# ariasanovsky/azdopt

Measured on AMD Instinct MI355X. Metric: node_expansions_per_s, higher is better.
Workload: dtype f32

## Files before the change

azdopt_amd/_lib.py:

```python
import ctypes as C
import os
import subprocess

_HERE = os.path.dirname(os.path.abspath(__file__))
LIB_PATH = os.environ.get("AZD_LIB", os.path.join(_HERE, "libazdopt_amd.so"))
_LIB = None

CTR = dict(EXPANSIONS=0, TERMINALS=1, TRANSPOSITIONS=2, VISITED_STEPS=3, SELECT_CALLS=4, SUM_DEG=5,
           SUM_ACTIONS=6, CASCADE_NODES=7, NEW_PREDS=8, ROOT_EXHAUSTED=9, MAX_FRONTIER=10, MAX_DEPTH=11,
           CURIOSITY_PAIRS=12, EVAL_LAYER_CLOCKS=13, TICKS_ADD_ACTIONS=14, FAILED=15, TICKS_TOTAL=16, TICKS_SELECT=17, TICKS_LOOKUP=18, TICKS_NEWNODE=19,
           TICKS_CASCADE=20, TICKS_MAX_CALL=21, TICKS_LAMBDA=22, TICKS_MATCHING=23, TICKS_WAIT=24, EVAL_BATCHES=25, EVAL_ROWS=26, EVAL_TILES=27, TICKS_TILES=28, TICKS_BATCH=29, TICKS_TILE_SETUP=30, TICKS_TILE_KLOOP=31)
CTR_COUNT = 32

ACT_NONE, ACT_RELU, ACT_SIGMOID = 0, 1, 2
ENGINE_NO_PERSISTENT_STEP = 1
ENGINE_ASYNC_STEP = 2
ENGINE_BARRIER_STEP = 4
ENGINE_POOL_STEP = 8
ENGINE_DENSE_AH = 32
ENGINE_RAMSEY_U64 = 16
ENGINE_EXT_POOL_STEP = 64
SPACE_C21 = 1
SPACE_RAMSEY = 2
SPACE_DENSE = 3
# ... 107 lines not shown
    sig("azd_evaluator_destroy", C.c_int, vp)
    sig("azd_evaluator_write_predictions", C.c_int, vp, C.c_int, vp, vp)
    sig("azd_evaluator_update_model", C.c_int, vp, C.c_int, vp, vp, vp, f32p)
    sig("azd_evaluator_write_predictions_dev", C.c_int, vp, C.c_int, vp, vp, vp)
    sig("azd_evaluator_update_model_dev", C.c_int, vp, C.c_int, vp, vp, vp, f32p, vp)
    sig("azd_evaluator_set_weight_storage", C.c_int, vp, C.c_int)
    sig("azd_evaluator_num_params", C.c_int64, vp)
    sig("azd_evaluator_get_params", C.c_int, vp, vp)
    sig("azd_evaluator_set_params", C.c_int, vp, vp)
    sig("azd_evaluator_calls", C.c_uint64, vp)
    sig("azd_engine_create", C.c_int, C.POINTER(vp), C.POINTER(EngineConfig), vp)
    sig("azd_engine_destroy", C.c_int, vp)
    sig("azd_engine_par_new", C.c_int, vp, vp, vp)
    sig("azd_engine_par_roll_out_episodes", C.c_int, vp, vp, C.c_int, C.c_uint32, C.c_int, i32p)
    sig("azd_engine_run_ahead", C.c_int, vp, vp, C.c_int, C.c_uint32, C.c_int, i32p)
    sig("azd_engine_par_update_model", C.c_int, vp, C.c_uint32, f32p)
    sig("azd_engine_par_update_model_sharded", C.c_int, vp, C.c_uint32, vp, f32p)
    sig("azd_engine_par_reset_trees", C.c_int, vp, vp, vp)
    sig("azd_engine_argmin_data", C.c_int, vp, C.POINTER(Argmin))
    sig("azd_engine_agent_counters", C.c_int, vp, vp)
    sig("azd_engine_agent_counters_per_agent", C.c_int, vp)
    sig("azd_engine_pool_agent_finish", C.c_int, vp, vp)
    sig("azd_engine_pool_groups", C.c_int, vp, vp, vp, vp)
    sig("azd_engine_ramsey_argmin_data", C.c_int, vp, C.POINTER(RamseyArgmin))
    sig("azd_engine_ramsey_wide_argmin_data", C.c_int, vp, C.POINTER(RamseyWideArgmin))
    sig("azd_engine_ramsey_argmin_any", C.c_int, vp, vp, C.c_int, vp, C.c_int, vp, f32p, i32p, C.POINTER(C.c_uint32))
    sig("azd_engine_ramsey_agent_counts", C.c_int, vp, C.c_int, vp, vp)
    sig("azd_ramsey_state_dim", C.c_int, C.c_int, C.c_int)
    sig("azd_ramsey_action_dim", C.c_int, C.c_int, C.c_int)
    sig("azd_ramsey_key_words", C.c_int, C.c_int, C.c_int)
    sig("azd_ramsey_generate_roots", C.c_int, C.c_uint64, C.c_uint64, C.c_uint64, C.c_int, C.c_int, C.c_int, C.c_int,
        C.c_int, vp, vp)
    sig("azd_ramsey_generate_roots_weighted", C.c_int, C.c_uint64, C.c_uint64, C.c_uint64, C.c_int, C.c_int, C.c_int, C.c_int,
        C.c_int, vp, vp, vp)
    sig("azd_engine_set_root_policy", C.c_int, vp, C.POINTER(RootPolicy))
    sig("azd_engine_get_root_policy", C.c_int, vp, C.POINTER(RootPolicy))
    sig("azd_root_policy_check", C.c_int, C.c_int, C.c_int, C.POINTER(RootPolicy))
    sig("azd_engine_root_policy_report", C.c_int, vp, vp, vp, vp)
    sig("azd_dense_state_dim", C.c_int, C.c_int)
    sig("azd_dense_action_dim", C.c_int, C.c_int)
    sig("azd_dense_key_words", C.c_int, C.c_int)
    sig("azd_dense_generate_roots", C.c_int, C.c_uint64, C.c_uint64, C.c_uint64, C.c_int, C.c_int, C.c_int, C.c_int, C.c_double, vp, vp)
    sig("azd_engine_dense_argmin_data", C.c_int, vp, C.POINTER(DenseArgmin))
    sig("azd_c21_modify_roots", C.c_int, vp, C.c_uint64, C.c_uint64, C.c_int, C.c_int, vp, vp)
    sig("azd_c21_modify_roots_dev", C.c_int, vp, C.c_uint64, C.c_uint64, C.c_int, C.c_int, vp, vp)
    sig("azd_engine_par_reset_trees_c21", C.c_int, vp, C.c_uint64, C.c_uint64, C.c_int, C.c_int)
# ... 47 lines not shown
```

azdopt_amd/csrc/async_step.inc:

```

struct AsyncCtl {
    uint32_t req[PERSIST_WAVES];
    uint32_t rows[PERSIST_WAVES];
    uint32_t nrows;
    uint32_t lock;
    uint32_t active;
    uint32_t gen;
    uint32_t tile_next[8];
    uint32_t tile_done[8];
    uint32_t finished;
    uint32_t prog[PERSIST_WAVES];
    unsigned long long t_open;
};

#define LDS_LOAD(p) __hip_atomic_load((p), __ATOMIC_RELAXED, __HIP_MEMORY_SCOPE_WORKGROUP)
#define LDS_STORE(p, v) __hip_atomic_store((p), (v), __ATOMIC_RELAXED, __HIP_MEMORY_SCOPE_WORKGROUP)
#define WG_RELEASE() __builtin_amdgcn_fence(__ATOMIC_RELEASE, "workgroup")
#define WG_ACQUIRE() __builtin_amdgcn_fence(__ATOMIC_ACQUIRE, "workgroup")

struct EvalPtrs {
    const void *__restrict__ wpk;
    const float *__restrict__ params;
    const float *state_vecs;
    float *h_theta;
};

__device__ __forceinline__ float *row_lds(const uint32_t owner_wave, const uint32_t dyn_stride) {
    return reinterpret_cast<float *>(lds_base(owner_wave * dyn_stride) + 16u * owner_wave);
}

typedef short bf16x4 __attribute__((ext_vector_type(4)));

struct AsyncRows {
    AsyncCtl &ctl;
    uint32_t dyn_stride;
    int t0;
    __device__ __forceinline__ int count() const { return (int)LDS_LOAD(&ctl.nrows); }
    __device__ __forceinline__ float *row(const int r) const { return row_lds(LDS_LOAD(&ctl.rows[r]), dyn_stride); }
    __device__ __forceinline__ int agent(const int r) const { return t0 + (int)LDS_LOAD(&ctl.rows[r]); }
    __device__ __forceinline__ float *out(const int) const { return nullptr; }
};

#ifndef AZD_MLP_PF
#define AZD_MLP_PF 8
#endif
constexpr int MLP_PF = AZD_MLP_PF;
template <class Rows, bool LAST_TO_LDS = false>
__device__ void mlp_tile_task(const FusedEval &ev, const Rows &rows, const EvalPtrs &gp, const int l, const int tile,
                              unsigned long long *ph) {
    ph[0] = PH_NOW();
    const int lane = LANE;
    const int L = ev.n_layers;
    const int K = ev.dims[l], N = ev.dims[l + 1];
    const int S4 = (ev.dims[0] + 15) & ~15, H = ev.hid[0];
    const int nrows = rows.count();
    const int n0 = tile * 16;
    const int r = lane & 15;
    const int rr = r < nrows ? r : 0;
    float *const rbase = rows.row(rr);
    const float *arow = rbase + (l == 0 ? 0 : S4 + ((l - 1) & 1) * H);
    const float *ap = arow + 4 * (lane >> 4);
    f32x4 acc = {0.f, 0.f, 0.f, 0.f};
    const int steps = (K + 15) >> 4;
    const size_t frag = (size_t)ev.p_off[l] + ((size_t)tile * steps * 64 + lane) * 4;
    ph[1] = PH_NOW();
    if (ev.bf16) {
        const uint16_t *wq = reinterpret_cast<const uint16_t *>(gp.wpk) + frag;
        const uint16_t *ap16 = reinterpret_cast<const uint16_t *>(rbase) + (l == 0 ? 0 : S4 + ((l - 1) & 1) * H) + 4 * (lane >> 4);
        int s0 = 0;
        for (; s0 + MLP_PF <= steps; s0 += MLP_PF) {
            uint2 bq[MLP_PF], aq[MLP_PF];
#pragma unroll
            for (int j = 0; j < MLP_PF; ++j) bq[j] = *reinterpret_cast<const uint2 *>(wq + 256 * (s0 + j));
#pragma unroll
            for (int j = 0; j < MLP_PF; ++j) aq[j] = *reinterpret_cast<const uint2 *>(ap16 + 16 * (s0 + j));
            __builtin_amdgcn_sched_barrier(0);
#pragma unroll
            for (int j = 0; j < MLP_PF; ++j) {
                bf16x4 a4, b4;
                __builtin_memcpy(&a4, &aq[j], 8);
                __builtin_memcpy(&b4, &bq[j], 8);
                acc = __builtin_amdgcn_mfma_f32_16x16x16bf16_1k(a4, b4, acc, 0, 0, 0);
            }
        }
        if (s0 < steps) {
            uint2 bq[MLP_PF];
#pragma unroll
            for (int j = 0; j < MLP_PF; ++j)
                if (s0 + j < steps) bq[j] = *reinterpret_cast<const uint2 *>(wq + 256 * (s0 + j));
            __builtin_amdgcn_sched_barrier(0);
#pragma unroll
            for (int j = 0; j < MLP_PF; ++j)
                if (s0 + j < steps) {
                    const uint2 bv = bq[j];
                    const uint2 ab = *reinterpret_cast<const uint2 *>(ap16 + 16 * (s0 + j));
                    bf16x4 a4, b4;
                    __builtin_memcpy(&a4, &ab, 8);
                    __builtin_memcpy(&b4, &bv, 8);
                    acc = __builtin_amdgcn_mfma_f32_16x16x16bf16_1k(a4, b4, acc, 0, 0, 0);
                }
        }
    } else {
        const float *wp = reinterpret_cast<const float *>(gp.wpk) + frag;
        int s0 = 0;
        for (; s0 + MLP_PF <= steps; s0 += MLP_PF) {
            float4 bq[MLP_PF];
#pragma unroll
            for (int j = 0; j < MLP_PF; ++j) bq[j] = *reinterpret_cast<const float4 *>(wp + 256 * (s0 + j));
            float4 a0 = *reinterpret_cast<const float4 *>(ap + 16 * s0);
            float4 a1 = *reinterpret_cast<const float4 *>(ap + 16 * (s0 + 1));
            __builtin_amdgcn_sched_barrier(0);
#pragma unroll
            for (int j = 0; j < MLP_PF; ++j) {
                float4 a2 = a1;
                if (j + 2 < MLP_PF) a2 = *reinterpret_cast<const float4 *>(ap + 16 * (s0 + j + 2));
                acc = __builtin_amdgcn_mfma_f32_16x16x4f32(a0.x, bq[j].x, acc, 0, 0, 0);
                acc = __builtin_amdgcn_mfma_f32_16x16x4f32(a0.y, bq[j].y, acc, 0, 0, 0);
                acc = __builtin_amdgcn_mfma_f32_16x16x4f32(a0.z, bq[j].z, acc, 0, 0, 0);
                acc = __builtin_amdgcn_mfma_f32_16x16x4f32(a0.w, bq[j].w, acc, 0, 0, 0);
                __builtin_amdgcn_sched_barrier(0);
                a0 = a1;
                a1 = a2;
            }
        }
        if (s0 < steps) {
            float4 bq[MLP_PF];
#pragma unroll
// ... 304 lines not shown
```

azdopt_amd/csrc/engine.hip:

```cpp
#include <hip/hip_runtime.h>

#include <dlfcn.h>

#include <algorithm>
#include <cstdio>
#include <cstring>
#include <new>
#include <string>
#include <vector>

#include "../../include/azdopt_amd.h"
#include "c21_host.h"
#include "engine_types.h"
#include "evaluator.h"
#include "space_ops.h"

namespace azd {

thread_local std::string g_last_error;

int hip_fail(hipError_t e, const char *what) {
    g_last_error = std::string(what) + ": " + hipGetErrorString(e);
    if (e == hipErrorNoDevice || e == hipErrorInvalidDevice) return AZD_ERR_NO_DEVICE;
    if (e == hipErrorOutOfMemory) return AZD_ERR_OUT_OF_MEMORY;
// ... 200 lines not shown
    unsigned long long *d_ext_t0 = nullptr;
    int ext_depth = 2;
    hipEvent_t ext_done = nullptr, ext_fork = nullptr, ext_ring[EXT_STREAMS][EXT_IN_FLIGHT] = {};
    unsigned long long ext_iterations = 0;
    const struct ExtPoolForm *ext = nullptr;
    uint16_t *ext_s16 = nullptr;
    int ext_s16_pitch = 0;
    int kw_host = 0;
    int ramsey_slots = 0;
    int dense_slots = 0;
    uint64_t *d_stage_slots = nullptr;
    azd_root_policy root_policy{AZD_ROOT_RULE_THRESHOLD, 0, {0.0, 0.0, 0.0, 0.0}};
    azd::RootPolicyArgs root_args{};
    uint32_t *d_root_report = nullptr;
    uint32_t *root_report = nullptr;
    bool root_report_valid = false;
    std::vector<uint64_t> dense_packed;
    std::vector<uint64_t> ramsey_perm_pad;
    bool pool_step = false;
    azd::PoolArgs pool{};
    size_t pool_slot_words = 0;
    int n_cus = 0;
    int pool_eval_wgs = 0, pool_search_wgs = 0;
    int pool_grp_g = 0, pool_grp_groups = 0, pool_grp_w = 0;
    int pool_search_waves = 0;
    double pool_util_eval = 0, pool_util_search = 0;
    struct {
        int n_eval = 0;
        int updates = 0;
    } pool_fb;
    struct Window {
        bool open = false;
        bool drained = false;
        bool lumped = false;
        int n = 0, consumed = 0;
        azd::TolTable tol{};
        uint32_t best_ord = 0;
        unsigned long long best_key = ~0ull;
        unsigned long long side_key = ~0ull;
        unsigned long long base_improved = 0;
        unsigned long long reported = 0;
        azd::FusedEval fe{};
        azd::PoolArgs pool{};
    } win;
    unsigned long long *h_win_log = nullptr;
    uint32_t *h_win_flag = nullptr;
// ... 1069 lines not shown
        e->step_reason = xf.r_no_wg;
        return AZD_OK;
    }
    int n_ext = xf.streams;
    if (const char *env = getenv(xf.env_streams)) n_ext = atoi(env);
    n_ext = n_ext < 1 ? 1 : n_ext > azd_engine::EXT_STREAMS ? azd_engine::EXT_STREAMS : n_ext;
    if (!e->ext_done) AZD_HIP(hipEventCreateWithFlags(&e->ext_done, hipEventDisableTiming));
    if (!e->ext_fork) AZD_HIP(hipEventCreateWithFlags(&e->ext_fork, hipEventDisableTiming));
    for (int x = 0; x < n_ext; ++x) {
        if (!e->ext_stream[x]) AZD_HIP(hipStreamCreateWithFlags(&e->ext_stream[x], hipStreamNonBlocking));
        for (int i = 0; i < azd_engine::EXT_IN_FLIGHT; ++i)
            if (!e->ext_ring[x][i]) AZD_HIP(hipEventCreateWithFlags(&e->ext_ring[x][i], hipEventDisableTiming));
    }
    azd::PoolArgs pool = e->pool;
    pool.n_eval = 0;
    pool.ready_lanes = 0;
    pool.n_express = 0;
    pool.express_waves = 0;
    pool.express_shift = 0;
    pool.early_post = xf.early_post;
    if (const char *env = getenv("AZD_POOL_EARLY_POST")) pool.early_post = atoi(env);
    pool.eval_stride = pool.eval_out_off = 0;
    pool.eval_rows = 0;
    pool.debug_abort_call = 0;
    if (const char *env = getenv("AZD_POOL_DEBUG_ABORT_CALL")) pool.debug_abort_call = (uint32_t)atoi(env);
    if (!hashed) {
        const int st_r = e->ev->ensure_rows(n_ext * a.B);
        if (st_r) return st_r;
    }
    int rounds = 4;
    if (const char *env = getenv(xf.env_rounds)) rounds = atoi(env);
    rounds = rounds < 1 ? 1 : rounds > 16 ? 16 : rounds;
    const uint64_t layout = e->ev->layout_version + (hashed ? 1ull << 63 : 0ull) + ((uint64_t)rounds << 56);
    if (e->ext_graph_n != n_ext || e->ext_graph_layout != layout) {
        for (int x = 0; x < azd_engine::EXT_STREAMS; ++x)
            if (e->ext_graph[x]) {
                (void)hipGraphExecDestroy(e->ext_graph[x]);
                e->ext_graph[x] = nullptr;
            }
        e->ext_graph_n = 0;
        for (int x = 0; x < n_ext; ++x) {
            uint32_t *rows = e->d_ext_rows + (size_t)x * a.B, *home = e->d_ext_home + (size_t)x * a.B, *cnt = e->d_ext_n + x;
            hipGraph_t g = nullptr;
            AZD_HIP(hipStreamBeginCapture(e->ext_stream[x], hipStreamCaptureModeThreadLocal));
            int st_g = AZD_OK;
            for (int r = 0; r < rounds && st_g == AZD_OK; ++r) {
// ... 224 lines not shown
            }
            n_eval = n_eval < 1 ? 1 : n_eval;
            if (pool_feedback_on() && e->pool_fb.n_eval > 0) {
                const int fb = e->pool_fb.n_eval;
                const int want_search = (B + 7) / 8, most = want_search < e->n_cus / 2 ? e->n_cus - want_search : e->n_cus / 2;
                n_eval = fb > cap ? cap : fb;
                n_eval = n_eval > most ? most : n_eval;
                n_eval = n_eval < 1 ? 1 : n_eval;
            }
            if (n_calls <= 64 && fe.kind == 3) {
                const int want_search = (B + 7) / 8, most = want_search < e->n_cus / 2 ? e->n_cus - want_search : e->n_cus / 2;
                n_eval += n_eval / 7;
                n_eval = n_eval > most ? most : n_eval;
                n_eval = n_eval > cap ? cap : n_eval;
            }
            if (const char *env = getenv("AZD_POOL_EVAL_WGS")) n_eval = atoi(env) > 0 ? atoi(env) : n_eval;
        }
        int n_search = e->n_cus - n_eval;
        const int want = (B + 7) / 8;
        n_search = n_search > want ? want : n_search;
        n_search = n_search < 1 ? 1 : n_search;
        if (const char *env = getenv("AZD_POOL_SEARCH_WGS")) n_search = atoi(env) > 0 ? atoi(env) : n_search;
        int capacity = e->ops->pool_max_resident(e->a, dyn_bytes, e->n_cus);
        if (const char *env = getenv("AZD_POOL_MAX_RESIDENT")) capacity = atoi(env);
        if (fe.kind < 3) n_eval = 0;
        if (n_eval + n_search > capacity) {
            if (n_eval > capacity / 2) n_eval = capacity / 2;
            if (fe.kind >= 3 && n_eval < 1) n_eval = 1;
            n_search = capacity - n_eval;
        }
        if (n_search < 1 || capacity < 1) {
            use_pool = false;
            char buf[160];
            snprintf(buf, sizeof(buf), "pool step: the device holds %d of its workgroups at once; it needs an evaluator and a searcher resident together; ", capacity);
            e->step_reason = buf;
        }
        pool.n_eval = n_eval;
        pool.ready_lanes = 0;
        if (const char *env = getenv("AZD_POOL_READY_LANES")) pool.ready_lanes = atoi(env);
        pool.n_express = (fe.kind >= 3 && n_search >= 64) ? 8 : 0;
        pool.express_waves = 8;
        pool.express_shift = 4;
        if (const char *env = getenv("AZD_POOL_EXPRESS_WGS")) pool.n_express = atoi(env);
        if (const char *env = getenv("AZD_POOL_EXPRESS_WAVES")) pool.express_waves = (uint32_t)atoi(env);
        if (const char *env = getenv("AZD_POOL_EXPRESS_SHIFT")) pool.express_shift = (uint32_t)atoi(env);
        if (pool.n_express > n_search / 2) pool.n_express = n_search / 2;
// ... 57 lines not shown
                    e->grp_lds_host = gpl.lds;
                }
                pool.grp_g = gpl.g;
                pool.grp_w = gpl.W;
                pool.grp_groups = n_groups;
                pool.grp_tile = e->d_grp_tile;
                pool.grp_lds = e->d_grp_lds;
                pool.grp_desc = e->d_grp_desc;
                pool.grp_cnt = e->d_grp_cnt;
                pool.grp_x = e->d_grp_x;
                pool.grp_flag = e->d_grp_flag;
                pool.grp_xstride = gpl.xstride;
                n_eval = n_groups * gpl.g;
                pool.n_eval = n_eval;
                if (gpl.lds_bytes > dyn_bytes) dyn_bytes = gpl.lds_bytes;
            }
        }
        pool_blocks = n_eval + n_search;
        e->pool_grp_g = pool.grp_g;
        e->pool_grp_groups = pool.grp_groups;
        e->pool_grp_w = pool.grp_w;
        e->pool_eval_wgs = n_eval;
        e->pool_search_wgs = n_search;
        e->pool_search_waves = (n_search - pool.n_express) * 16 + pool.n_express * (int)pool.express_waves;
    }
    if (e->pool_step && fusable && !use_pool) {
        use_async = !e->barrier_step && e->ops->async_plan(e->a, fe, &dyn_stride, &dyn_bytes, &why_a);
        use_barrier = !use_async && e->ops->persist_plan(e->a, fe, &dyn_stride, &dyn_bytes, &why_b);
        if (!use_async) e->step_reason += why_a;
        if (!use_async && !use_barrier && *why_b) e->step_reason += std::string("; ") + why_b;
    }
    e->step_form = use_pool ? AZD_STEP_POOL : use_async ? AZD_STEP_ASYNC : use_barrier ? AZD_STEP_BARRIER : AZD_STEP_PER_CALL;
    if (e->a.space == azd::SPACE_DENSE)
        e->step_reason = dense_reason.empty() ? "AZD_DENSE_NO_POOL: the dense-graph space's pool step was switched off" : dense_reason;
    if (ext_ramsey) e->step_reason = ext_demoted || e->step_reason.empty() ? ext_reason : ext_reason + "; " + e->step_reason;
    if (ahead) {
        const bool ok = use_pool && fe.kind >= 3 && n_calls >= 1 && n_calls <= e->log_calls && !e->timing;
        if (!ok) return AZD_OK;
        *accepted = 1;
    }
    if (use_pool || use_async || use_barrier) {
        auto send_args = [&](const azd::PoolArgs &pl) -> int {
            azd::PersistArgs &pa = e->pargs_sent;
            azd::PersistArgs now;
            memset(&now, 0, sizeof(now));
            now.a = e->a;
// ... 1028 lines not shown
    return AZD_OK;
}
int azd_engine_timing(azd_engine *e, double *tree_ms, double *evaluator_ms, uint64_t *tree_launches) {
    if (!e) return AZD_ERR_INVALID_ARGUMENT;
    if (tree_ms) *tree_ms = e->rollout_ms;
    if (evaluator_ms) *evaluator_ms = e->evaluator_ms;
    if (tree_launches) *tree_launches = e->rollout_launches;
    return AZD_OK;
}
void *azd_engine_stream(azd_engine *e) { return e ? (void *)e->stream : nullptr; }
int azd_engine_pool_utilisation(azd_engine *e, double *eval_busy, double *search_busy) {
    if (!e) return AZD_ERR_INVALID_ARGUMENT;
    if (eval_busy) *eval_busy = e->pool_util_eval;
    if (search_busy) *search_busy = e->pool_util_search;
    return AZD_OK;
}
int azd_engine_pool_groups(azd_engine *e, int *members, int *groups, int *waves_per_slot) {
    if (!e) return AZD_ERR_INVALID_ARGUMENT;
    if (members) *members = e->pool_grp_g;
    if (groups) *groups = e->pool_grp_groups;
    if (waves_per_slot) *waves_per_slot = e->pool_grp_w;
    return AZD_OK;
}
int azd_engine_pool_agent_finish(azd_engine *e, uint64_t *ticks_out) {
    if (!e || !ticks_out) return AZD_ERR_INVALID_ARGUMENT;
    AZD_ENTER(e);
    if (!e->pool.stamp) {
        azd::g_last_error = "pool_agent_finish: this engine has run no pool step";
        return AZD_ERR_INVALID_ARGUMENT;
    }
    AZD_HIP(hipStreamSynchronize(e->stream));
    AZD_HIP(hipMemcpy(ticks_out, e->pool.stamp, (size_t)e->a.B * 8, hipMemcpyDeviceToHost));
    return AZD_OK;
}
int azd_engine_pool_split(azd_engine *e, int *eval_wgs, int *search_wgs) {
    if (!e) return AZD_ERR_INVALID_ARGUMENT;
    if (eval_wgs) *eval_wgs = e->pool_eval_wgs;
    if (search_wgs) *search_wgs = e->pool_search_wgs;
    return AZD_OK;
}
int azd_debug_probe_xcc(int device, uint32_t *out, int n_blocks) {
    if (!out || n_blocks <= 0) return AZD_ERR_INVALID_ARGUMENT;
    int st = azd::device_ok(device);
    if (st) return st;
    AZD_HIP(hipSetDevice(device));
    uint32_t *d = nullptr;
// ... 271 lines not shown
```

azdopt_amd/csrc/engine_types.h:

```cpp
#pragma once
#include <stddef.h>
#include <stdint.h>

namespace azd {

constexpr uint32_t NONE = 0xFFFFFFFFu;
constexpr int PARENTS_STRIDE = 32;
constexpr int MAX_N = 24;
constexpr int MAX_KW = 6;
constexpr int PATH_SET = 0, PATH_SEQUENCE = 1;
constexpr int SPACE_C21 = 1, SPACE_RAMSEY = 2, SPACE_DENSE = 3;
constexpr int PRED_CHUNKS = 2;
constexpr int MAX_NODE_ACTIONS = 64 * PRED_CHUNKS;
constexpr int RAMSEY_U64_KW = 36;
constexpr int RAMSEY_U64_CH = 8;
constexpr int FRONTIER_CAP = 256;
constexpr int PATH_STACK = 32;
constexpr int MAX_TOL = 32;
constexpr int NUM_COUNTERS = 32;

struct __attribute__((aligned(16))) NodeRec {
    float c_star;
    uint32_t nt_ex;
    float c;
// ... 224 lines not shown
struct PendRec {
    uint32_t pos;
    float c;
    uint32_t n_preds;
    uint32_t call;
};
struct PoolArgs {
    PoolCtl *ctl;
    uint32_t *ready_slots;
    uint32_t *eval_slots;
    int ready_lanes;
    int n_express;
    uint32_t express_waves;
    uint32_t express_shift;
    int early_post;
    uint32_t qcap;
    uint32_t *join;
    PendRec *pend;
    unsigned long long *stamp;
    int n_eval;
    uint32_t eval_stride;
    uint32_t eval_out_off;
    uint32_t eval_rows;
    uint32_t *post_call;
    int grp_g, grp_w, grp_groups;
    const int16_t *grp_tile;
    const uint32_t *grp_lds;
    uint32_t *grp_desc;
    uint32_t *grp_cnt;
    uint32_t *grp_flag;
    float *grp_x;
    uint32_t grp_xstride;
    uint32_t debug_abort_call;
    uint32_t *win_count;
    unsigned long long *win_log;
    uint32_t *win_flag;
};

struct StepLaunch {
    int n_calls;
    unsigned long long *log_key;
    const uint32_t *resume;
    PoolCtl *ctl;
    int hashed;
    int groups = 0;
    int window;
// ... 11 lines not shown
```

azdopt_amd/csrc/pool_step.inc:

```

constexpr unsigned long long POOL_WAIT_TICKS = 400000000ull;
struct PoolWait {
    unsigned long long t0;
    uint32_t polls;
    __device__ __forceinline__ PoolWait() : t0(0), polls(0) {}
    __device__ __forceinline__ bool expired() {
        if ((++polls & 255u) != 0u) return false;
        const unsigned long long now = (unsigned long long)wall_clock64();
        if (t0 == 0) t0 = now;
        return now - t0 > POOL_WAIT_TICKS;
    }
};

__device__ __forceinline__ uint32_t pool_xcc_id() {
    uint32_t v;
    asm volatile("s_getreg_b32 %0, hwreg(HW_REG_XCC_ID)" : "=s"(v));
    return v & 7u;
}

#ifndef AZD_POOL_FILL_WAIT
#define AZD_POOL_FILL_WAIT 2
#endif
#ifndef AZD_POOL_FILL_SLEEP
#define AZD_POOL_FILL_SLEEP 32
// ... 29 lines not shown
#define POOL_FLUSH_PER_AGENT(A, S, T) ((void)0)
#endif
#ifndef AZD_POOL_EXPRESS_SLACK
#define AZD_POOL_EXPRESS_SLACK 2
#endif
#ifndef AZD_POOL_STANDBY
#define AZD_POOL_STANDBY 4
#endif
constexpr int POOL_BATCH_MAX = 32;
struct PoolBatch {
    uint32_t agent[POOL_BATCH_MAX];
    uint32_t home[POOL_BATCH_MAX];
    uint32_t n, first[2], cnt[2], q, leave;
};

struct PoolRows {
    uint32_t stride, out_off;
    const uint32_t *agents;
    int n;
    __device__ __forceinline__ int count() const { return n; }
    __device__ __forceinline__ float *row(const int r) const { return reinterpret_cast<float *>(lds_base((uint32_t)r * stride * 4u)); }
    __device__ __forceinline__ int agent(const int r) const { return (int)agents[r]; }
    __device__ __forceinline__ float *out(const int r) const { return reinterpret_cast<float *>(lds_base(((uint32_t)r * stride + out_off) * 4u)); }
};

template <bool BF16>
__device__ void pool_tile2(const FusedEval &ev, const PoolRows &rows, const EvalPtrs &gp, const int l, const int tile) {
    const int lane = LANE;
    const int L = ev.n_layers;
    const int K = ev.dims[l], N = ev.dims[l + 1];
    const int S4 = (ev.dims[0] + 15) & ~15, H = ev.hid[0];
    const int nrows = rows.count();
    const int n0 = tile * 16;
    const int r = lane & 15;
    float *const base0 = rows.row(r < nrows ? r : 0);
    float *const base1 = rows.row(16 + r < nrows ? 16 + r : 0);
    const int in_off = (l == 0 ? 0 : S4 + ((l - 1) & 1) * H) + 4 * (lane >> 4);
    const int steps = (K + 15) >> 4;
    const size_t frag = (size_t)ev.p_off[l] + ((size_t)tile * steps * 64 + lane) * 4;
    f32x4 acc0 = {0.f, 0.f, 0.f, 0.f}, acc1 = {0.f, 0.f, 0.f, 0.f};
    if constexpr (BF16) {
        const uint16_t *wq = reinterpret_cast<const uint16_t *>(gp.wpk) + frag;
        const uint16_t *p0 = reinterpret_cast<const uint16_t *>(base0) + in_off, *p1 = reinterpret_cast<const uint16_t *>(base1) + in_off;
        for (int s0 = 0; s0 < steps; s0 += MLP_PF) {
            uint2 bq[MLP_PF];
            const bool full = s0 + MLP_PF <= steps;
#pragma unroll
            for (int j = 0; j < MLP_PF; ++j)
                if (full || s0 + j < steps) bq[j] = *reinterpret_cast<const uint2 *>(wq + 256 * (s0 + j));
            __builtin_amdgcn_sched_barrier(0);
#pragma unroll
            for (int j = 0; j < MLP_PF; ++j)
                if (full || s0 + j < steps) {
                    const uint2 a0 = *reinterpret_cast<const uint2 *>(p0 + 16 * (s0 + j)), a1 = *reinterpret_cast<const uint2 *>(p1 + 16 * (s0 + j));
                    bf16x4 x0, x1, b4;
                    __builtin_memcpy(&x0, &a0, 8);
                    __builtin_memcpy(&x1, &a1, 8);
                    __builtin_memcpy(&b4, &bq[j], 8);
                    acc0 = __builtin_amdgcn_mfma_f32_16x16x16bf16_1k(x0, b4, acc0, 0, 0, 0);
                    acc1 = __builtin_amdgcn_mfma_f32_16x16x16bf16_1k(x1, b4, acc1, 0, 0, 0);
                }
        }
    } else {
        const float *wp = reinterpret_cast<const float *>(gp.wpk) + frag;
        const float *p0 = base0 + in_off, *p1 = base1 + in_off;
        for (int s0 = 0; s0 < steps; s0 += MLP_PF) {
            float4 bq[MLP_PF];
            const bool full = s0 + MLP_PF <= steps;
#pragma unroll
            for (int j = 0; j < MLP_PF; ++j)
                if (full || s0 + j < steps) bq[j] = *reinterpret_cast<const float4 *>(wp + 256 * (s0 + j));
            __builtin_amdgcn_sched_barrier(0);
#pragma unroll
            for (int j = 0; j < MLP_PF; ++j)
                if (full || s0 + j < steps) {
                    const float4 a0 = *reinterpret_cast<const float4 *>(p0 + 16 * (s0 + j)), a1 = *reinterpret_cast<const float4 *>(p1 + 16 * (s0 + j));
                    acc0 = __builtin_amdgcn_mfma_f32_16x16x4f32(a0.x, bq[j].x, acc0, 0, 0, 0);
                    acc1 = __builtin_amdgcn_mfma_f32_16x16x4f32(a1.x, bq[j].x, acc1, 0, 0, 0);
                    acc0 = __builtin_amdgcn_mfma_f32_16x16x4f32(a0.y, bq[j].y, acc0, 0, 0, 0);
                    acc1 = __builtin_amdgcn_mfma_f32_16x16x4f32(a1.y, bq[j].y, acc1, 0, 0, 0);
                    acc0 = __builtin_amdgcn_mfma_f32_16x16x4f32(a0.z, bq[j].z, acc0, 0, 0, 0);
                    acc1 = __builtin_amdgcn_mfma_f32_16x16x4f32(a1.z, bq[j].z, acc1, 0, 0, 0);
                    acc0 = __builtin_amdgcn_mfma_f32_16x16x4f32(a0.w, bq[j].w, acc0, 0, 0, 0);
                    acc1 = __builtin_amdgcn_mfma_f32_16x16x4f32(a1.w, bq[j].w, acc1, 0, 0, 0);
                }
        }
    }
    const int col = n0 + (lane & 15);
    if (col < N) {
// ... 61 lines not shown
                                            const int A) {
    for (int idx = threadIdx.x; idx < n * A; idx += PERSIST_WAVES * 64) {
        const int r = idx / A, i = idx - r * A;
        const uint64_t agent = ev.first_agent + (uint64_t)bt.agent[r], cidx = ev.call_base + (uint64_t)ld_sc1(pl.post_call + bt.agent[r]);
        const uint64_t h = splitmix(splitmix(splitmix(splitmix(ev.seed ^ 0x70726564ull) ^ agent) ^ cidx) ^ (uint64_t)i);
        rows.out(r)[i] = (float)(h >> 40) * (1.0f / 16777216.0f);
    }
}

template <bool HASHED>
__device__ __forceinline__ void pool_eval(const PersistArgs *pa, const EvalPtrs &gp, PoolBatch &bt, const uint32_t xcc) {
    const Arenas &a = pa->a;
    const FusedEval &ev = pa->ev;
    const PoolArgs &pl = pa->pool;
    PoolCtl *ctl = pl.ctl;
    const int tid = threadIdx.x, wave = tid >> 6;
    const uint32_t B = (uint32_t)a.B, qmask = pl.qcap - 1u;
    constexpr bool hashed = HASHED;
    const int S = ev.dims[0], S16 = (S + 15) & ~15, L = hashed ? 0 : ev.n_layers, A = hashed ? a.A : ev.dims[L];
    PoolRows rows;
    rows.stride = pl.eval_stride;
    rows.out_off = pl.eval_out_off;
    rows.agents = bt.agent;
    unsigned long long n_batches = 0, n_rows = 0, n_tiles = 0, busy = 0, t_stage = 0, t_layers = 0, c_layers = 0;
    for (;;) {
        if (tid == 0) {
            uint32_t n = 0, first0 = 0, first1 = 0, cnt0 = 0, cnt1 = 0, q = 0, leave = 0;
            PoolWait wt;
            int fill_waits = AZD_POOL_FILL_WAIT;
            for (;;) {
                for (uint32_t k = 0; k < (uint32_t)POOL_XCDS && n == 0u; ++k) {
                    const uint32_t x = (xcc + k) & (uint32_t)(POOL_XCDS - 1);
                    const uint32_t h0 = AZD_POOL_PRIORITY ? ld_sc1(&ctl->evalq[0][x].head) : 0u, t0 = AZD_POOL_PRIORITY ? ld_sc1(&ctl->evalq[0][x].tail) : 0u;
                    const uint32_t h1 = ld_sc1(&ctl->evalq[1][x].head), t1 = ld_sc1(&ctl->evalq[1][x].tail);
                    const int a0 = (int)(t0 - h0) > 0 ? (int)(t0 - h0) : 0, a1 = (int)(t1 - h1) > 0 ? (int)(t1 - h1) : 0;
                    if (a0 + a1 == 0) continue;
                    const int cap = ((int)pl.eval_rows > PERSIST_WAVES && a0 + a1 >= (int)pl.eval_rows) ? (int)pl.eval_rows : PERSIST_WAVES;
                    if (a0 == 0 && a1 < PERSIST_WAVES && fill_waits > 0) {
                        --fill_waits;
                        __builtin_amdgcn_s_sleep(AZD_POOL_FILL_SLEEP);
                        k = (uint32_t)POOL_XCDS;
                        continue;
                    }
                    uint32_t c0 = 0, c1 = 0;
                    if (a0 > 0) {
                        const uint32_t take = a0 < cap ? (uint32_t)a0 : (uint32_t)cap;
// ... 867 lines not shown
        const uint64_t h = splitmix(splitmix(splitmix(splitmix(ev.seed ^ 0x70726564ull) ^ agent) ^ cidx) ^ (uint64_t)i);
        h_theta[(size_t)t * A + i] = (float)(h >> 40) * (1.0f / 16777216.0f);
    }
}
#endif

static bool pool_plan_common(const Arenas &a, const FusedEval &ev, PoolArgs *pool, uint32_t *dyn_stride, size_t *dyn_bytes,
                             const char **why, const size_t search_bytes, const size_t wave_lds_bytes) {
    if (a.B > 65536 || a.node_cap > 65536) {
        *why = "pool step: more than 65536 agents or nodes per tree";
        return false;
    }
    if (a.S % 4 != 0) {
        *why = "pool step: STATE_DIM must be a multiple of 4 (rows travel as 16-byte stores)";
        return false;
    }
    const size_t stride = (search_bytes + 15) & ~(size_t)15;
    const size_t sw_bytes = (PERSIST_WAVES * wave_lds_bytes + 15) & ~(size_t)15;
    size_t total = sw_bytes + stride * PERSIST_WAVES;
    const size_t static_lds = sizeof(PoolBatch) + sizeof(PoolIdle) + 256;
    pool->eval_stride = 0;
    pool->eval_out_off = 0;
    pool->eval_rows = PERSIST_WAVES;
    if (ev.kind == 3) {
        for (int l = 0; l < ev.n_layers; ++l)
            if (ev.dims[l] % (l == 0 ? 4 : 16) != 0) {
                *why = "pool step: hidden widths must be multiples of 16 and the input width a multiple of 4";
                return false;
            }
        const int A = ev.dims[ev.n_layers];
        if (A % 4 != 0) {
            *why = "pool step: ACTION_DIM must be a multiple of 4 (rows travel as 16-byte stores)";
            return false;
        }
        const size_t x_el = (size_t)((ev.dims[0] + 15) & ~15);
        const size_t act = x_el + (size_t)ev.hid[0] + (size_t)ev.hid[1];
        const size_t act_fl = ev.bf16 ? act / 2 : act;
        const size_t x_fl = ev.bf16 ? x_el / 2 : x_el;
        const bool alias = ev.n_layers >= 2 && (size_t)A <= x_fl;
        const size_t out_off = alias ? 0 : act_fl;
        const size_t row = act_fl + (alias ? 0 : (size_t)A) + 4;
        pool->eval_stride = (uint32_t)row;
        pool->eval_out_off = (uint32_t)out_off;
        const bool two = AZD_POOL_TWO_TILES && row * sizeof(float) * POOL_BATCH_MAX + static_lds <= 160 * 1024;
        pool->eval_rows = two ? POOL_BATCH_MAX : PERSIST_WAVES;
        const size_t eval_bytes = row * sizeof(float) * pool->eval_rows;
        if (eval_bytes > total) total = eval_bytes;
    }
    if (ev.kind == 4) {
        if (a.A % 4 != 0) {
            *why = "pool step: ACTION_DIM must be a multiple of 4 (rows travel as 16-byte stores)";
            return false;
        }
        pool->eval_stride = (uint32_t)a.A + 4u;
        pool->eval_out_off = 0;
        pool->eval_rows = POOL_BATCH_MAX;
        const size_t eval_bytes = (size_t)pool->eval_stride * sizeof(float) * pool->eval_rows;
        if (eval_bytes > total) total = eval_bytes;
    }
    if (total + static_lds > 160 * 1024) {
        *why = "pool step: a batch of 16 rows (or 16 searcher waves' blocks and scratch) does not fit the CU's 160 KB of LDS";
        return false;
    }
    *dyn_stride = (uint32_t)stride;
    *dyn_bytes = total;
    return true;
}
```

azdopt_amd/optimizer.py:

```python
import ctypes as C

import numpy as np

from . import _lib
from .space import ActionSet


class ArgminData:

    def __init__(self, rec, n, kw):
        self.state = dict(parents=np.array(rec.parents[:n], np.uint8), permitted=np.array(rec.permitted[:kw], np.uint64))
        m = rec.matching_size
        self.cost = dict(lambda_1=rec.lambda_1, matching=[(rec.matching[2 * i], rec.matching[2 * i + 1]) for i in range(m)])
        self.eval = np.float32(rec.eval)
        self.agent, self.node = rec.agent, rec.node


class RamseyArgminData:

    def __init__(self, rec, space):
        self.state = dict(colors=np.array(rec.colors[:space.E], np.uint8), permitted=np.array(rec.permitted[:], np.uint64))
        self.cost = dict(clique_counts=[int(x) for x in rec.totals[:space.C]])
        self.eval = np.float32(rec.eval)
        self.agent, self.node = rec.agent, rec.node
# ... 304 lines not shown
        counts = np.zeros((self.space.C, self.space.E), np.int32)
        totals = np.zeros(4, np.int32)
        _lib.check(self._L.azd_engine_ramsey_agent_counts(self._h, agent, _lib.ptr(counts), _lib.ptr(totals)), "ramsey_agent_counts")
        return counts, totals[:self.space.C]

    def counters(self):
        out = np.zeros(_lib.CTR_COUNT, np.uint64)
        _lib.check(self._L.azd_engine_counters(self._h, _lib.ptr(out)), "counters")
        return {k: int(out[v]) for k, v in _lib.CTR.items()}

    def agent_counters(self, allow_wave_blocks=False):
        if not allow_wave_blocks and self._L.azd_engine_agent_counters_per_agent(self._h) == 0:
            raise RuntimeError("agent_counters: the pool step of the product build attributes counters to searcher waves, not agents "
                               "(use counters() for the sums, the PROFILE build or pool_step=False for per-agent values)")
        out = np.zeros((self.batch, _lib.CTR_COUNT), np.uint64)
        _lib.check(self._L.azd_engine_agent_counters(self._h, _lib.ptr(out)), "agent_counters")
        return {k: out[:, v].copy() for k, v in _lib.CTR.items()}

    def pool_groups(self):
        g, n, w = C.c_int(), C.c_int(), C.c_int()
        _lib.check(self._L.azd_engine_pool_groups(self._h, C.byref(g), C.byref(n), C.byref(w)), "pool_groups")
        return g.value, n.value, w.value

    def pool_agent_finish_ms(self):
        out = np.zeros(self.batch, np.uint64)
        _lib.check(self._L.azd_engine_pool_agent_finish(self._h, _lib.ptr(out)), "pool_agent_finish")
        return out.astype(np.float64) * 1e-5

    def set_timing(self, enabled=True):
        _lib.check(self._L.azd_engine_set_timing(self._h, int(enabled)), "set_timing")

    def timing(self):
        a, b, n = C.c_double(), C.c_double(), C.c_uint64()
        _lib.check(self._L.azd_engine_timing(self._h, C.byref(a), C.byref(b), C.byref(n)), "timing")
        return dict(rollout_ms=a.value, evaluator_ms=b.value, rollout_launches=n.value)

    def stream(self):
        return self._L.azd_engine_stream(self._h)

    STEP_FORMS = {0: "none", 1: "async", 2: "barrier", 3: "per_call", 4: "pool", 5: "per_call_graph"}

    def pool_split(self):
        a, b = C.c_int32(), C.c_int32()
        _lib.check(self._L.azd_engine_pool_split(self._h, C.byref(a), C.byref(b)), "pool_split")
        return a.value, b.value

# ... 10 lines not shown
```

include/azdopt_amd.h:

```cpp
#ifndef AZDOPT_AMD_H
#define AZDOPT_AMD_H
#include <stdint.h>
#ifdef __cplusplus
extern "C" {
#endif

typedef enum azd_status {
    AZD_OK = 0,
    AZD_ERR_INVALID_ARGUMENT = 1,
    AZD_ERR_NO_DEVICE = 2,
    AZD_ERR_HIP = 3,
    AZD_ERR_CAPACITY = 4,
    AZD_ERR_UNREACHABLE = 5,
    AZD_ERR_NO_EVALUATOR = 6,
    AZD_ERR_OUT_OF_MEMORY = 7,
    AZD_ERR_UNSUPPORTED = 8
} azd_status;

const char *azd_status_string(int status);
const char *azd_last_error(void);
int azd_version(void);
int azd_device_count(void);

#define AZD_SPACE_C21 1
// ... 233 lines not shown

int azd_engine_tree_sizes(azd_engine *e, int agent, int *n_nodes, int *n_arcs, int *n_predictions);
int azd_engine_export_tree(azd_engine *e, int agent, float *c, float *c_star, uint32_t *n_t,
                           uint32_t *exhausted, uint32_t *act_begin, uint32_t *act_end,
                           uint64_t *keys, uint32_t *arc_src, uint32_t *arc_dst, uint32_t *arc_pp,
                           uint32_t *pred_a_id, float *pred_g, int32_t *pred_arc);
int azd_engine_agent_state(azd_engine *e, int agent, uint8_t *parents, uint64_t *permitted,
                           uint64_t *path, uint32_t *state_pos, double *lambda_1,
                           int *matching_size);
int azd_engine_counters(azd_engine *e, uint64_t *out );
int azd_engine_agent_counters(azd_engine *e, uint64_t *out);
int azd_engine_agent_counters_per_agent(azd_engine *e);
int azd_engine_set_timing(azd_engine *e, int enabled);
int azd_engine_timing(azd_engine *e, double *tree_ms, double *evaluator_ms, uint64_t *tree_launches);
void *azd_engine_stream(azd_engine *e);
#define AZD_STEP_NONE 0
#define AZD_STEP_ASYNC 1
#define AZD_STEP_BARRIER 2
#define AZD_STEP_PER_CALL 3
#define AZD_STEP_POOL 4
#define AZD_STEP_PER_CALL_GRAPH 5
int azd_engine_step_form(azd_engine *e, int *form, const char **reason);
int azd_engine_pool_groups(azd_engine *e, int *members, int *groups, int *waves_per_slot);
int azd_engine_pool_agent_finish(azd_engine *e, uint64_t *ticks_out);
int azd_engine_pool_split(azd_engine *e, int *eval_wgs, int *search_wgs);
int azd_engine_pool_utilisation(azd_engine *e, double *eval_busy, double *search_busy);
int azd_debug_probe_xcc(int device, uint32_t *out, int n_blocks);
int azd_debug_hash_stream_via_evaluators(azd_evaluator *ev, int on);
int azd_debug_ext_pool_plan(const azd_engine_config *cfg, int *waves, size_t *lds_bytes);
int azd_debug_mlp_gradients(azd_evaluator *ev, int batch, const float *states, const float *observations,
                            const float *action_weights, float *grads_out, float *loss);

int azd_debug_probe_math(int device, const float *in, float *out, int n);
int azd_debug_probe_cost(int device, const uint8_t *parents, int n, int count, int reps, int full,
                         double *lambda_1, int *matching_size, float *ms);

#define AZD_DENSE_AH_MAX_N 32
typedef struct azd_dense_ah_cost_t {
    double proximity;
    double eigenvalue;
    int32_t diameter;
    int32_t k;
    float cost;
    float eval;
} azd_dense_ah_cost_t;
int azd_dense_ah_cost(const uint64_t *adj, int n, azd_dense_ah_cost_t *out);
// ... 22 lines not shown
```

Measured before the change: 38.76 million.

## Keep MLP weight fragments resident in LDS for persistent pool evaluator workgroups

Pool evaluator workgroups now copy as many per-layer weight fragments as fit in spare LDS once at startup, and the MFMA tile loops read those steps from LDS before falling back to global memory for the rest. This targets repeated global and L2 weight fetches on every batch. It enlarges dynamic LDS per workgroup, which can lower residency. The host therefore drops the resident weights if they would reduce capacity below the needed workgroup count, and may switch from two-tile to single-tile batches to free room.

```diff
diff --git a/azdopt_amd/_lib.py b/azdopt_amd/_lib.py
--- a/azdopt_amd/_lib.py
+++ b/azdopt_amd/_lib.py
@@ -153,6 +153,7 @@
     sig("azd_engine_agent_counters_per_agent", C.c_int, vp)
     sig("azd_engine_pool_agent_finish", C.c_int, vp, vp)
     sig("azd_engine_pool_groups", C.c_int, vp, vp, vp, vp)
+    sig("azd_engine_pool_resident", C.c_int, vp, vp, vp)
     sig("azd_engine_ramsey_argmin_data", C.c_int, vp, C.POINTER(RamseyArgmin))
     sig("azd_engine_ramsey_wide_argmin_data", C.c_int, vp, C.POINTER(RamseyWideArgmin))
     sig("azd_engine_ramsey_argmin_any", C.c_int, vp, vp, C.c_int, vp, C.c_int, vp, f32p, i32p, C.POINTER(C.c_uint32))
diff --git a/azdopt_amd/csrc/async_step.inc b/azdopt_amd/csrc/async_step.inc
--- a/azdopt_amd/csrc/async_step.inc
+++ b/azdopt_amd/csrc/async_step.inc
@@ -39,6 +39,7 @@
     __device__ __forceinline__ float *row(const int r) const { return row_lds(LDS_LOAD(&ctl.rows[r]), dyn_stride); }
     __device__ __forceinline__ int agent(const int r) const { return t0 + (int)LDS_LOAD(&ctl.rows[r]); }
     __device__ __forceinline__ float *out(const int) const { return nullptr; }
+    static constexpr bool RESIDENT = false;
 };
 
 #ifndef AZD_MLP_PF
@@ -63,11 +64,35 @@
     f32x4 acc = {0.f, 0.f, 0.f, 0.f};
     const int steps = (K + 15) >> 4;
     const size_t frag = (size_t)ev.p_off[l] + ((size_t)tile * steps * 64 + lane) * 4;
+    int rs = 0;
+    uint32_t wl = 0;
+    if constexpr (Rows::RESIDENT) {
+        rs = rows.resident_steps(l, steps);
+        wl = rows.resident_tile(l, tile, rs, ev.bf16 ? 2u : 4u) + (uint32_t)lane * (ev.bf16 ? 8u : 16u);
+    }
     ph[1] = PH_NOW();
     if (ev.bf16) {
         const uint16_t *wq = reinterpret_cast<const uint16_t *>(gp.wpk) + frag;
         const uint16_t *ap16 = reinterpret_cast<const uint16_t *>(rbase) + (l == 0 ? 0 : S4 + ((l - 1) & 1) * H) + 4 * (lane >> 4);
-        int s0 = 0;
+        if constexpr (Rows::RESIDENT)
+            for (int g = 0; g < rs; g += MLP_PF) {
+                uint2 bq[MLP_PF];
+#pragma unroll
+                for (int j = 0; j < MLP_PF; ++j)
+                    if (g + j < rs) bq[j] = *reinterpret_cast<const uint2 *>(lds_base(wl + 512u * (uint32_t)(g + j)));
+                __builtin_amdgcn_sched_barrier(0);
+#pragma unroll
+                for (int j = 0; j < MLP_PF; ++j)
+                    if (g + j < rs) {
+                        const uint2 bv = bq[j];
+                        const uint2 ab = *reinterpret_cast<const uint2 *>(ap16 + 16 * (g + j));
+                        bf16x4 a4, b4;
+                        __builtin_memcpy(&a4, &ab, 8);
+                        __builtin_memcpy(&b4, &bv, 8);
+                        acc = __builtin_amdgcn_mfma_f32_16x16x16bf16_1k(a4, b4, acc, 0, 0, 0);
+                    }
+            }
+        int s0 = rs;
         for (; s0 + MLP_PF <= steps; s0 += MLP_PF) {
             uint2 bq[MLP_PF], aq[MLP_PF];
 #pragma unroll
@@ -102,7 +127,25 @@
         }
     } else {
         const float *wp = reinterpret_cast<const float *>(gp.wpk) + frag;
-        int s0 = 0;
+        if constexpr (Rows::RESIDENT)
+            for (int g = 0; g < rs; g += MLP_PF) {
+                float4 bq[MLP_PF];
+#pragma unroll
+                for (int j = 0; j < MLP_PF; ++j)
+                    if (g + j < rs) bq[j] = *reinterpret_cast<const float4 *>(lds_base(wl + 1024u * (uint32_t)(g + j)));
+                __builtin_amdgcn_sched_barrier(0);
+#pragma unroll
+                for (int j = 0; j < MLP_PF; ++j)
+                    if (g + j < rs) {
+                        const float4 bv = bq[j];
+                        const float4 av = *reinterpret_cast<const float4 *>(ap + 16 * (g + j));
+                        acc = __builtin_amdgcn_mfma_f32_16x16x4f32(av.x, bv.x, acc, 0, 0, 0);
+                        acc = __builtin_amdgcn_mfma_f32_16x16x4f32(av.y, bv.y, acc, 0, 0, 0);
+                        acc = __builtin_amdgcn_mfma_f32_16x16x4f32(av.z, bv.z, acc, 0, 0, 0);
+                        acc = __builtin_amdgcn_mfma_f32_16x16x4f32(av.w, bv.w, acc, 0, 0, 0);
+                    }
+            }
+        int s0 = rs;
         for (; s0 + MLP_PF <= steps; s0 += MLP_PF) {
             float4 bq[MLP_PF];
 #pragma unroll
diff --git a/azdopt_amd/csrc/engine.hip b/azdopt_amd/csrc/engine.hip
--- a/azdopt_amd/csrc/engine.hip
+++ b/azdopt_amd/csrc/engine.hip
@@ -246,6 +246,7 @@
     size_t pool_slot_words = 0;
     int n_cus = 0;
     int pool_eval_wgs = 0, pool_search_wgs = 0;
+    unsigned pool_res_bytes = 0, pool_batch_rows = 0;
     int pool_grp_g = 0, pool_grp_groups = 0, pool_grp_w = 0;
     int pool_search_waves = 0;
     double pool_util_eval = 0, pool_util_search = 0;
@@ -1361,6 +1362,7 @@
     if (const char *env = getenv("AZD_POOL_EARLY_POST")) pool.early_post = atoi(env);
     pool.eval_stride = pool.eval_out_off = 0;
     pool.eval_rows = 0;
+    pool.eval_res_bytes = pool.eval_dyn_min = 0;
     pool.debug_abort_call = 0;
     if (const char *env = getenv("AZD_POOL_DEBUG_ABORT_CALL")) pool.debug_abort_call = (uint32_t)atoi(env);
     if (!hashed) {
@@ -1631,6 +1633,14 @@
         n_search = n_search < 1 ? 1 : n_search;
         if (const char *env = getenv("AZD_POOL_SEARCH_WGS")) n_search = atoi(env) > 0 ? atoi(env) : n_search;
         int capacity = e->ops->pool_max_resident(e->a, dyn_bytes, e->n_cus);
+        if (pool.eval_res_bytes != 0u && dyn_bytes > pool.eval_dyn_min && n_eval + n_search > capacity) {
+            const int cap0 = e->ops->pool_max_resident(e->a, pool.eval_dyn_min, e->n_cus);
+            if (cap0 > capacity) {
+                pool.eval_res_bytes = 0;
+                dyn_bytes = pool.eval_dyn_min;
+                capacity = cap0;
+            }
+        }
         if (const char *env = getenv("AZD_POOL_MAX_RESIDENT")) capacity = atoi(env);
         if (fe.kind < 3) n_eval = 0;
         if (n_eval + n_search > capacity) {
@@ -1734,6 +1744,8 @@
         e->pool_grp_w = pool.grp_w;
         e->pool_eval_wgs = n_eval;
         e->pool_search_wgs = n_search;
+        e->pool_res_bytes = pool.eval_res_bytes;
+        e->pool_batch_rows = pool.eval_rows;
         e->pool_search_waves = (n_search - pool.n_express) * 16 + pool.n_express * (int)pool.express_waves;
     }
     if (e->pool_step && fusable && !use_pool) {
@@ -2808,6 +2820,12 @@
     if (waves_per_slot) *waves_per_slot = e->pool_grp_w;
     return AZD_OK;
 }
+int azd_engine_pool_resident(azd_engine *e, unsigned *weight_bytes, unsigned *batch_rows) {
+    if (!e) return AZD_ERR_INVALID_ARGUMENT;
+    if (weight_bytes) *weight_bytes = e->pool_res_bytes;
+    if (batch_rows) *batch_rows = e->pool_batch_rows;
+    return AZD_OK;
+}
 int azd_engine_pool_agent_finish(azd_engine *e, uint64_t *ticks_out) {
     if (!e || !ticks_out) return AZD_ERR_INVALID_ARGUMENT;
     AZD_ENTER(e);
diff --git a/azdopt_amd/csrc/engine_types.h b/azdopt_amd/csrc/engine_types.h
--- a/azdopt_amd/csrc/engine_types.h
+++ b/azdopt_amd/csrc/engine_types.h
@@ -270,6 +270,10 @@
     uint32_t eval_stride;
     uint32_t eval_out_off;
     uint32_t eval_rows;
+    uint32_t eval_res_bytes;
+    uint32_t eval_res_loff[7];
+    uint16_t eval_res_steps[8];
+    uint32_t eval_dyn_min;
     uint32_t *post_call;
     int grp_g, grp_w, grp_groups;
     const int16_t *grp_tile;
diff --git a/azdopt_amd/csrc/pool_step.inc b/azdopt_amd/csrc/pool_step.inc
--- a/azdopt_amd/csrc/pool_step.inc
+++ b/azdopt_amd/csrc/pool_step.inc
@@ -75,6 +75,17 @@
     __device__ __forceinline__ float *row(const int r) const { return reinterpret_cast<float *>(lds_base((uint32_t)r * stride * 4u)); }
     __device__ __forceinline__ int agent(const int r) const { return (int)agents[r]; }
     __device__ __forceinline__ float *out(const int r) const { return reinterpret_cast<float *>(lds_base(((uint32_t)r * stride + out_off) * 4u)); }
+    static constexpr bool RESIDENT = true;
+    const uint16_t *res_steps = nullptr;
+    const uint32_t *res_loff = nullptr;
+    __device__ __forceinline__ int resident_steps(const int l, const int steps) const {
+        if (res_steps == nullptr) return 0;
+        const int have = (int)res_steps[l];
+        return have < steps ? have : steps;
+    }
+    __device__ __forceinline__ uint32_t resident_tile(const int l, const int tile, const int rs, const uint32_t esz) const {
+        return rs > 0 ? res_loff[l] + (uint32_t)(tile * rs) * 256u * esz : 0u;
+    }
 };
 
 template <bool BF16>
@@ -92,10 +103,30 @@
     const int steps = (K + 15) >> 4;
     const size_t frag = (size_t)ev.p_off[l] + ((size_t)tile * steps * 64 + lane) * 4;
     f32x4 acc0 = {0.f, 0.f, 0.f, 0.f}, acc1 = {0.f, 0.f, 0.f, 0.f};
+    const int rs = rows.resident_steps(l, steps);
+    const uint32_t wl = rows.resident_tile(l, tile, rs, BF16 ? 2u : 4u) + (uint32_t)lane * (BF16 ? 8u : 16u);
     if constexpr (BF16) {
         const uint16_t *wq = reinterpret_cast<const uint16_t *>(gp.wpk) + frag;
         const uint16_t *p0 = reinterpret_cast<const uint16_t *>(base0) + in_off, *p1 = reinterpret_cast<const uint16_t *>(base1) + in_off;
-        for (int s0 = 0; s0 < steps; s0 += MLP_PF) {
+        for (int g = 0; g < rs; g += MLP_PF) {
+            uint2 bq[MLP_PF];
+#pragma unroll
+            for (int j = 0; j < MLP_PF; ++j)
+                if (g + j < rs) bq[j] = *reinterpret_cast<const uint2 *>(lds_base(wl + 512u * (uint32_t)(g + j)));
+            __builtin_amdgcn_sched_barrier(0);
+#pragma unroll
+            for (int j = 0; j < MLP_PF; ++j)
+                if (g + j < rs) {
+                    const uint2 a0 = *reinterpret_cast<const uint2 *>(p0 + 16 * (g + j)), a1 = *reinterpret_cast<const uint2 *>(p1 + 16 * (g + j));
+                    bf16x4 x0, x1, b4;
+                    __builtin_memcpy(&x0, &a0, 8);
+                    __builtin_memcpy(&x1, &a1, 8);
+                    __builtin_memcpy(&b4, &bq[j], 8);
+                    acc0 = __builtin_amdgcn_mfma_f32_16x16x16bf16_1k(x0, b4, acc0, 0, 0, 0);
+                    acc1 = __builtin_amdgcn_mfma_f32_16x16x16bf16_1k(x1, b4, acc1, 0, 0, 0);
+                }
+        }
+        for (int s0 = rs; s0 < steps; s0 += MLP_PF) {
             uint2 bq[MLP_PF];
             const bool full = s0 + MLP_PF <= steps;
 #pragma unroll
@@ -117,7 +148,27 @@
     } else {
         const float *wp = reinterpret_cast<const float *>(gp.wpk) + frag;
         const float *p0 = base0 + in_off, *p1 = base1 + in_off;
-        for (int s0 = 0; s0 < steps; s0 += MLP_PF) {
+        for (int g = 0; g < rs; g += MLP_PF) {
+            float4 bq[MLP_PF];
+#pragma unroll
+            for (int j = 0; j < MLP_PF; ++j)
+                if (g + j < rs) bq[j] = *reinterpret_cast<const float4 *>(lds_base(wl + 1024u * (uint32_t)(g + j)));
+            __builtin_amdgcn_sched_barrier(0);
+#pragma unroll
+            for (int j = 0; j < MLP_PF; ++j)
+                if (g + j < rs) {
+                    const float4 a0 = *reinterpret_cast<const float4 *>(p0 + 16 * (g + j)), a1 = *reinterpret_cast<const float4 *>(p1 + 16 * (g + j));
+                    acc0 = __builtin_amdgcn_mfma_f32_16x16x4f32(a0.x, bq[j].x, acc0, 0, 0, 0);
+                    acc1 = __builtin_amdgcn_mfma_f32_16x16x4f32(a1.x, bq[j].x, acc1, 0, 0, 0);
+                    acc0 = __builtin_amdgcn_mfma_f32_16x16x4f32(a0.y, bq[j].y, acc0, 0, 0, 0);
+                    acc1 = __builtin_amdgcn_mfma_f32_16x16x4f32(a1.y, bq[j].y, acc1, 0, 0, 0);
+                    acc0 = __builtin_amdgcn_mfma_f32_16x16x4f32(a0.z, bq[j].z, acc0, 0, 0, 0);
+                    acc1 = __builtin_amdgcn_mfma_f32_16x16x4f32(a1.z, bq[j].z, acc1, 0, 0, 0);
+                    acc0 = __builtin_amdgcn_mfma_f32_16x16x4f32(a0.w, bq[j].w, acc0, 0, 0, 0);
+                    acc1 = __builtin_amdgcn_mfma_f32_16x16x4f32(a1.w, bq[j].w, acc1, 0, 0, 0);
+                }
+        }
+        for (int s0 = rs; s0 < steps; s0 += MLP_PF) {
             float4 bq[MLP_PF];
             const bool full = s0 + MLP_PF <= steps;
 #pragma unroll
@@ -225,6 +276,23 @@
     rows.stride = pl.eval_stride;
     rows.out_off = pl.eval_out_off;
     rows.agents = bt.agent;
+    if (!hashed && pl.eval_res_bytes != 0u) {
+        rows.res_steps = pl.eval_res_steps;
+        rows.res_loff = pl.eval_res_loff;
+        const uint32_t qb = ev.bf16 ? 8u : 16u;
+        for (int l = 0; l < L; ++l) {
+            const uint32_t steps = (uint32_t)((ev.dims[l] + 15) >> 4), nt = (uint32_t)((ev.dims[l + 1] + 15) >> 4);
+            const uint32_t r = (uint32_t)rows.resident_steps(l, (int)steps);
+            const char *src = reinterpret_cast<const char *>(gp.wpk) + (size_t)ev.p_off[l] * (qb >> 2);
+            for (uint32_t q = (uint32_t)tid; q < nt * r * 64u; q += (uint32_t)(PERSIST_WAVES * 64)) {
+                const uint32_t ts = q >> 6, t = ts / r, st = ts - t * r;
+                const char *from = src + ((size_t)(t * steps + st) * 64u + (q & 63u)) * qb;
+                char *to = lds_base(pl.eval_res_loff[l] + q * qb);
+                if (ev.bf16) *reinterpret_cast<uint2 *>(to) = *reinterpret_cast<const uint2 *>(from);
+                else *reinterpret_cast<azd_f32x4 *>(to) = *reinterpret_cast<const azd_f32x4 *>(from);
+            }
+        }
+    }
     unsigned long long n_batches = 0, n_rows = 0, n_tiles = 0, busy = 0, t_stage = 0, t_layers = 0, c_layers = 0;
     for (;;) {
         if (tid == 0) {
@@ -1138,6 +1206,9 @@
     pool->eval_stride = 0;
     pool->eval_out_off = 0;
     pool->eval_rows = PERSIST_WAVES;
+    pool->eval_res_bytes = pool->eval_dyn_min = 0;
+    for (int l = 0; l < 7; ++l) pool->eval_res_loff[l] = pool->eval_res_steps[l] = 0;
+    pool->eval_res_steps[7] = 0;
     if (ev.kind == 3) {
         for (int l = 0; l < ev.n_layers; ++l)
             if (ev.dims[l] % (l == 0 ? 4 : 16) != 0) {
@@ -1160,8 +1231,41 @@
         pool->eval_out_off = (uint32_t)out_off;
         const bool two = AZD_POOL_TWO_TILES && row * sizeof(float) * POOL_BATCH_MAX + static_lds <= 160 * 1024;
         pool->eval_rows = two ? POOL_BATCH_MAX : PERSIST_WAVES;
-        const size_t eval_bytes = row * sizeof(float) * pool->eval_rows;
+        size_t eval_bytes = row * sizeof(float) * pool->eval_rows;
         if (eval_bytes > total) total = eval_bytes;
+        const char *env = getenv("AZD_POOL_RESIDENT_WEIGHTS");
+        if (!(env && atoi(env) == 0)) {
+            const size_t most = (size_t)160 * 1024 - static_lds;
+            const size_t room = (total + static_lds > 80 * 1024 && most > total) ? most : total;
+            const size_t step_bytes = 256 * (size_t)(ev.bf16 ? 2 : 4);
+            auto resident = [&](const size_t rows_bytes, PoolArgs *out) {
+                const size_t off = (rows_bytes + 15) & ~(size_t)15;
+                size_t left = off < room ? (room - off) / step_bytes : 0, at = off;
+                for (int l = 0; l < ev.n_layers; ++l) {
+                    const size_t steps = (size_t)((ev.dims[l] + 15) >> 4), nt = (size_t)((ev.dims[l + 1] + 15) >> 4);
+                    const size_t r = left / nt < steps ? left / nt : steps;
+                    if (out) {
+                        out->eval_res_steps[l] = (uint16_t)r;
+                        out->eval_res_loff[l] = (uint32_t)at;
+                    }
+                    left -= r * nt;
+                    at += r * nt * step_bytes;
+                }
+                return at - off;
+            };
+            if (two && a.B < 6144 && resident(eval_bytes / 2, nullptr) > resident(eval_bytes, nullptr)) {
+                pool->eval_rows = PERSIST_WAVES;
+                eval_bytes /= 2;
+            }
+            const size_t bytes = resident(eval_bytes, nullptr);
+            if (bytes > 0) {
+                resident(eval_bytes, pool);
+                pool->eval_res_bytes = (uint32_t)bytes;
+                pool->eval_dyn_min = (uint32_t)total;
+                const size_t end = ((eval_bytes + 15) & ~(size_t)15) + bytes;
+                if (end > total) total = end;
+            }
+        }
     }
     if (ev.kind == 4) {
         if (a.A % 4 != 0) {
diff --git a/azdopt_amd/optimizer.py b/azdopt_amd/optimizer.py
--- a/azdopt_amd/optimizer.py
+++ b/azdopt_amd/optimizer.py
@@ -350,6 +350,11 @@
         _lib.check(self._L.azd_engine_pool_groups(self._h, C.byref(g), C.byref(n), C.byref(w)), "pool_groups")
         return g.value, n.value, w.value
 
+    def pool_resident(self):
+        b, r = C.c_uint(), C.c_uint()
+        _lib.check(self._L.azd_engine_pool_resident(self._h, C.byref(b), C.byref(r)), "pool_resident")
+        return b.value, r.value
+
     def pool_agent_finish_ms(self):
         out = np.zeros(self.batch, np.uint64)
         _lib.check(self._L.azd_engine_pool_agent_finish(self._h, _lib.ptr(out)), "pool_agent_finish")
diff --git a/include/azdopt_amd.h b/include/azdopt_amd.h
--- a/include/azdopt_amd.h
+++ b/include/azdopt_amd.h
@@ -279,6 +279,7 @@
 #define AZD_STEP_PER_CALL_GRAPH 5
 int azd_engine_step_form(azd_engine *e, int *form, const char **reason);
 int azd_engine_pool_groups(azd_engine *e, int *members, int *groups, int *waves_per_slot);
+int azd_engine_pool_resident(azd_engine *e, unsigned *weight_bytes, unsigned *batch_rows);
 int azd_engine_pool_agent_finish(azd_engine *e, uint64_t *ticks_out);
 int azd_engine_pool_split(azd_engine *e, int *eval_wgs, int *search_wgs);
 int azd_engine_pool_utilisation(azd_engine *e, double *eval_busy, double *search_busy);
```

Result: no change. 38.65 million (-0.3%).
